# sitzikbs/Nesti-Net

Hardware: AMD Instinct MI355X
Metric: normals/sec (whole node), synthetic 100k-pt clouds (higher is better)
Workload: dtype f16x8c

## Files before the change

### nesti-net_amd/csrc/conv4n.hip

```cpp
#include <type_traits>

#include "kernels.h"
#include "mma.h"

namespace nesti {
namespace {

constexpr int kThreads4 = 512;
constexpr int kPts4 = 16;
constexpr int kTile4 = 1024;
constexpr int kBTap4 = 4 * kTile4;
constexpr int kABuf4 = 64 * kTile4;
constexpr int kEpiStride4 = 144;
constexpr int kEpi4 = 1024 * kEpiStride4;
template <int K> constexpr bool dba4() { return 2 * K * kBTap4 + 2 * kABuf4 <= 163840; }
template <int K> constexpr int lds4() {
  constexpr int loop = 2 * K * kBTap4 + (dba4<K>() ? 2 : 1) * kABuf4;
  return loop > kEpi4 ? loop : kEpi4;
}
constexpr unsigned kOob4 = 0x40000u;

typedef unsigned u32x4q_t __attribute__((ext_vector_type(4)));
typedef const __attribute__((address_space(3))) u32x4q_t* lds_u32x4q_ptr;
__device__ __forceinline__ uint4 lds128q(unsigned addr) {
  const u32x4q_t v = *(lds_u32x4q_ptr)(size_t)addr;
  return make_uint4(v.x, v.y, v.z, v.w);
}

typedef __attribute__((ext_vector_type(4))) float f32x4;
template <int DT> __device__ __forceinline__ void mma16(f32x4& acc, const uint4& a, const uint4& b);
template <> __device__ __forceinline__ void mma16<NESTI_BF16>(f32x4& acc, const uint4& a, const uint4& b) {
  acc = __builtin_amdgcn_mfma_f32_16x16x32_bf16(__builtin_bit_cast(bf16x8, a), __builtin_bit_cast(bf16x8, b), acc, 0, 0, 0);
}
template <> __device__ __forceinline__ void mma16<NESTI_F16>(f32x4& acc, const uint4& a, const uint4& b) {
  acc = __builtin_amdgcn_mfma_f32_16x16x32_f16(__builtin_bit_cast(f16x8, a), __builtin_bit_cast(f16x8, b), acc, 0, 0, 0);
}
template <> __device__ __forceinline__ void mma16<NESTI_F32>(f32x4& acc, const uint4& a, const uint4& b) {
  acc = __builtin_amdgcn_mfma_f32_16x16x4f32(__uint_as_float(a.x), __uint_as_float(b.x), acc, 0, 0, 0);
  acc = __builtin_amdgcn_mfma_f32_16x16x4f32(__uint_as_float(a.y), __uint_as_float(b.y), acc, 0, 0, 0);
  acc = __builtin_amdgcn_mfma_f32_16x16x4f32(__uint_as_float(a.z), __uint_as_float(b.z), acc, 0, 0, 0);
  acc = __builtin_amdgcn_mfma_f32_16x16x4f32(__uint_as_float(a.w), __uint_as_float(b.w), acc, 0, 0, 0);
}

__device__ __forceinline__ int swz4(int r) { return (0x78 >> (2 * ((r >> 2) & 3))) & 3; }

template <int DT, int K, bool X3>
__device__ __forceinline__ void conv4n_tile(const ConvParams& p, const unsigned bid, const int tid_in) {
  extern __shared__ __attribute__((aligned(16))) unsigned char smem[];
  constexpr int kEsz = (DT == NESTI_F32) ? 4 : 2;
  constexpr int NB = X3 ? 2 : 1;
  constexpr int LO = (K - 1) / 2;
  constexpr int NR = K * K;
  constexpr bool PREF = !X3 && K == 4;
  static_assert(K >= 2 && K <= 5, "kernel edge");
  constexpr bool DBA = dba4<K>();
  constexpr int kSlotB = K * kBTap4;
  constexpr int kAOff = 2 * kSlotB;
  constexpr int APR = NR >= 6 ? 4 : 2;
  constexpr int APP = 8 / APR;
  static_assert(lds4<K>() <= 163840, "LDS budget");

  const int tid = tid_in, lane = tid & 63;
  const int wave = __builtin_amdgcn_readfirstlane(tid >> 6);
  const int cw = wave & 3, h = wave >> 2;

  const int xcd = bid & 7, grp = bid >> 3;
  const int n_tile = grp % p.n_tiles;
  const int m_tile = (grp / p.n_tiles) * 8 + xcd;
  if (m_tile >= p.m_tiles) return;
  int npts = p.npoints;
  if (p.npoints_ptr) npts = min(npts, *p.npoints_ptr);
  const int p0 = m_tile * kPts4;
  if (p0 >= npts) return;
  const int np_here = min(kPts4, npts - p0);

  const unsigned lds0 = (unsigned)(size_t)(lptr_t)smem;
  const unsigned char* in_b = reinterpret_cast<const unsigned char*>(p.in) + ((size_t)p0 * 64 * p.in_cstride + p.in_coff) * kEsz;
  const unsigned char* w_tile = reinterpret_cast<const unsigned char*>(p.wpk) + (size_t)n_tile * p.n_chunks * (K * K * K) * kBTap4;

  const int st_row = lane >> 2;
  const int st_slot = (lane & 3) ^ swz4(st_row);
  const bool st_ok = st_row < np_here;
  const size_t st_off = (size_t)st_row * 64 * p.in_cstride * kEsz +
                        (X3 ? (size_t)((st_slot & 1) * 16 + (st_slot >> 1) * (2 * kSplitGroup)) : (size_t)st_slot * 16);
  auto stage_a = [&](int c, int buf, int q0, int nq) __attribute__((always_inline)) {
    const size_t coff = X3 ? (size_t)(c >> 2) * (2 * kPairPlanes * kSplitGroup) + (size_t)(c & 3) * 32
                           : p.in_pair ? (size_t)(c >> 1) * (2 * kPairPlanes * kSplitGroup) + (size_t)(c & 1) * 64 : (size_t)c * 64;
#pragma unroll
    for (int qq = 0; qq < nq; ++qq) {
      const int s = wave * 8 + q0 + qq;
      const int x = s & 3, z = (s >> 2) & 3, y = ((s >> 4) - z) & 3;
      const int v = 16 * z + 4 * y + x;
      if (st_ok) glds16(in_b + (size_t)v * p.in_cstride * kEsz + coff + st_off, lds0 + kAOff + buf * kABuf4 + s * kTile4);
    }
  };
  auto stage_b = [&](int g) __attribute__((always_inline)) {
    const unsigned char* src = w_tile + (size_t)g * kSlotB;
    for (int pid = wave; pid < 4 * K; pid += 8) glds16(src + pid * 1024 + lane * 16, lds0 + (g & 1) * kSlotB + pid * 1024);
  };

  const int r16 = lane & 15, kb = lane >> 4;
  const unsigned frag = (unsigned)(r16 * 64 + ((kb ^ swz4(r16)) << 4));
  const unsigned a_lane = lds0 + kAOff + frag;
  unsigned b_lane[NB];
  if (X3) {
    b_lane[0] = lds0 + (unsigned)(r16 * 64 + (((kb & 1) ^ swz4(r16)) << 4));
    b_lane[NB - 1] = kb < 2 ? lds0 + (unsigned)(r16 * 64 + (((2 + (kb & 1)) ^ swz4(r16)) << 4)) : kOob4;
  } else {
    b_lane[0] = lds0 + frag;
  }

  unsigned ymk = 0u, zmk = 0u;
#pragma unroll
  for (int d = 0; d < 5; ++d)
#pragma unroll
    for (int j = 0; j < 2; ++j) {
      const int z = 2 * h + j, y = (cw - z) & 3;
      if ((unsigned)(y + d - 2) < 4u) ymk |= 1u << (2 * d + j);
      if ((unsigned)(z + d - 2) < 4u) zmk |= 1u << (2 * d + j);
    }
  auto row_info = [&](int iz, int iy, int buf, unsigned& live, unsigned& abase) __attribute__((always_inline)) {
    const int dz = iz - LO, dy = iy - LO;
    live = (zmk >> (2 * (dz + 2))) & (ymk >> (2 * (dy + 2))) & 3u;
    const int tile0 = 4 * (4 * ((cw + dy + dz) & 3) + 2 * h + dz);
    abase = a_lane + (unsigned)(buf * kABuf4 + tile0 * kTile4);
  };

  f32x4 acc[2][4][4];
#pragma unroll
  for (int j = 0; j < 2; ++j)
#pragma unroll
    for (int x = 0; x < 4; ++x)
#pragma unroll
      for (int n = 0; n < 4; ++n)
#pragma unroll
        for (int r = 0; r < 4; ++r) acc[j][x][n][r] = 0.f;

  uint4 a[2][4], an[2][4], b[2][4][NB];
  auto load_a = [&](uint4 (&dst)[2][4], unsigned base) __attribute__((always_inline)) {
#pragma unroll
    for (int j = 0; j < 2; ++j)
#pragma unroll
      for (int x = 0; x < 4; ++x) dst[j][x] = lds128q(base + (4 * j + x) * kTile4);
  };
  auto load_b = [&](uint4 (&dst)[4][NB], unsigned off) __attribute__((always_inline)) {
#pragma unroll
    for (int n = 0; n < 4; ++n)
#pragma unroll
      for (int s = 0; s < NB; ++s) dst[n][s] = lds128q(b_lane[s] + off + n * kTile4);
  };

  const int G = p.n_chunks * NR;
  stage_a(0, 0, 0, 8);
  stage_b(0);
  stage_b(1);
  wait_vm0();
  __syncthreads();
  unsigned live_c, abase_c;
  row_info(0, 0, 0, live_c, abase_c);
  load_b(b[K & 1], 0u);
  if (PREF) load_a(an, abase_c);
  int c = 0, row = 0, iz = 0, iy = 0;
  for (int g = 0; g < G; ++g) {
    int cn = c, rown = row + 1, izn = iz, iyn = iy + 1;
    if (iyn == K) { iyn = 0; ++izn; }
    if (rown == NR) { rown = 0; izn = 0; iyn = 0; ++cn; }
    unsigned live_n = 0u, abase_n = abase_c;
    if (g + 1 < G) row_info(izn, iyn, DBA ? (cn & 1) : 0, live_n, abase_n);
    const bool stage_now = DBA && row < APR && c + 1 < p.n_chunks;
    if (stage_now) stage_a(c + 1, (c + 1) & 1, row * APP, APP);
    if (!PREF) {
      load_a(a, abase_c);
    } else {
#pragma unroll
      for (int j = 0; j < 2; ++j)
#pragma unroll
        for (int x = 0; x < 4; ++x) a[j][x] = an[j][x];
      load_a(an, abase_n);
    }
    const unsigned lv = live_c;
    const unsigned slot_off = (unsigned)((g & 1) * kSlotB), nslot_off = (unsigned)(((g + 1) & 1) * kSlotB);
#pragma unroll
    for (int u = 0; u < K; ++u) {
      const bool last = (u == K - 1);
      if ((K & 1) && u == 0) {
#pragma unroll
        for (int n = 0; n < 4; ++n)
#pragma unroll
          for (int s = 0; s < NB; ++s) b[0][n][s] = b[1][n][s];
      }
      uint4(&bc)[4][NB] = b[u & 1];
      uint4(&bn)[4][NB] = b[(u + 1) & 1];
      if (last) {
        __builtin_amdgcn_s_waitcnt(0xC07F);
        if (stage_now) asm volatile("s_waitcnt vmcnt(%0)" ::"n"(APP) : "memory");
        else wait_vm0();
        __builtin_amdgcn_s_barrier();
        if (g + 2 < G) stage_b(g + 2);
        if (!DBA && rown == 0 && g + 1 < G) {
          stage_a(cn, 0, 0, 8);
        }
      }
      load_b(bn, last ? nslot_off : slot_off + (unsigned)((u + 1) * kBTap4));
#pragma unroll
      for (int j = 0; j < 2; ++j) {
        if (__builtin_expect((lv & (1u << j)) != 0, 1)) {
#pragma unroll
          for (int x = 0; x < 4; ++x) {
            const int xs = x + u - LO;
            if (xs >= 0 && xs < 4) {
#pragma unroll
              for (int s = 0; s < NB; ++s)
#pragma unroll
                for (int n = 0; n < 4; ++n) mma16<DT>(acc[j][x][n], a[j][xs], bc[n][s]);
            }
          }
        }
      }
    }
    if (!DBA && rown == 0 && g + 1 < G) {
      wait_vm0();
      __builtin_amdgcn_s_barrier();
    }
    live_c = live_n;
    abase_c = abase_n;
    c = cn; row = rown; iz = izn; iy = iyn;
  }
  __builtin_amdgcn_s_waitcnt(0xC07F);
  __syncthreads();

  const int out_esz = p.out_f32 ? 4 : kEsz;
  const float act_floor = p.relu ? 0.f : -INFINITY;
  unsigned char* out_b = reinterpret_cast<unsigned char*>(p.out);
  unsigned char* mp_b = reinterpret_cast<unsigned char*>(p.mp_out);
  auto cvt_store8 = [&](unsigned char* base, long long row_elems, int col, const float4& f0, const float4& f1) __attribute__((always_inline)) {
    if (out_esz == 4) {
      float4* dst = reinterpret_cast<float4*>(base + (row_elems + col) * 4);
      dst[0] = f0;
      dst[1] = f1;
    } else {
      using E = Elem<DT == NESTI_F32 ? NESTI_BF16 : DT>;
      store_act8<E>(base, row_elems, col, f0, f1, p.split);
    }
  };
  auto epi_pass = [&](auto PP) __attribute__((always_inline)) {
    constexpr int pass = decltype(PP)::value;
    const int out_col0 = p.out_coff + n_tile * 64 + pass * 32;
#pragma unroll
    for (int n2 = 0; n2 < 2; ++n2) {
      const int n = 2 * pass + n2;
      const float bv = p.bias[n_tile * 64 + n * 16 + r16];
#pragma unroll
      for (int j = 0; j < 2; ++j) {
        const int z = 2 * h + j, y = (cw - z) & 3;
#pragma unroll
        for (int x = 0; x < 4; ++x) {
          const int v = 16 * z + 4 * y + x;
#pragma unroll
          for (int r = 0; r < 4; ++r) {
            const int row = (4 * kb + r) * 64 + v;
            *reinterpret_cast<float*>(smem + row * kEpiStride4 + (n2 * 16 + r16) * 4) = fmaxf(fmaf(acc[j][x][n][r], p.acc_scale, bv), act_floor);
          }
        }
      }
    }
    __syncthreads();
    if (p.mp_mode != 1) {
#pragma unroll 2
      for (int it = 0; it < 8; ++it) {
        const int item = it * kThreads4 + tid;
        const int row = item >> 2, seg = item & 3;
        const int ptl = row >> 6, vox = row & 63;
        if (ptl < np_here) {
          const float4 f0 = *reinterpret_cast<const float4*>(smem + row * kEpiStride4 + seg * 32);
          const float4 f1 = *reinterpret_cast<const float4*>(smem + row * kEpiStride4 + seg * 32 + 16);
          cvt_store8(out_b, ((long long)(p0 + ptl) * 64 + vox) * p.out_cstride, out_col0 + seg * 8, f0, f1);
        }
      }
    }
    if (p.mp_mode != 0) {
      const int cell = tid >> 2, seg = tid & 3;
      const int ptl = cell >> 3, cz = (cell >> 2) & 1, cy = (cell >> 1) & 1, cx = cell & 1;
      float4 m0 = make_float4(-INFINITY, -INFINITY, -INFINITY, -INFINITY), m1 = m0;
#pragma unroll
      for (int q = 0; q < 8; ++q) {
        const int row = ptl * 64 + (2 * cz + (q >> 2)) * 16 + (2 * cy + ((q >> 1) & 1)) * 4 + 2 * cx + (q & 1);
        const float4 f0 = *reinterpret_cast<const float4*>(smem + row * kEpiStride4 + seg * 32);
        const float4 f1 = *reinterpret_cast<const float4*>(smem + row * kEpiStride4 + seg * 32 + 16);
        m0.x = fmaxf(m0.x, f0.x); m0.y = fmaxf(m0.y, f0.y); m0.z = fmaxf(m0.z, f0.z); m0.w = fmaxf(m0.w, f0.w);
        m1.x = fmaxf(m1.x, f1.x); m1.y = fmaxf(m1.y, f1.y); m1.z = fmaxf(m1.z, f1.z); m1.w = fmaxf(m1.w, f1.w);
      }
      if (ptl < np_here)
        cvt_store8(mp_b, ((long long)(p0 + ptl) * 8 + (cz * 4 + cy * 2 + cx)) * p.mp_cstride, out_col0 + seg * 8, m0, m1);
    }
    __syncthreads();
  };
  epi_pass(std::integral_constant<int, 0>{});
  epi_pass(std::integral_constant<int, 1>{});
}

template <int DT, int K, bool X3, bool WALK>
__global__ __launch_bounds__(kThreads4) void conv4n_kernel(const ConvParams p) {
  if constexpr (!WALK) {
    conv4n_tile<DT, K, X3>(p, blockIdx.x, threadIdx.x);
  } else {
    unsigned n_blocks;
    {
      int npts = p.npoints;
      if (p.npoints_ptr) npts = min(npts, *p.npoints_ptr);
      const unsigned m_live = (unsigned)((npts + kPts4 - 1) / kPts4);
        n_blocks = (m_live + 7) / 8 * 8 * (unsigned)p.n_tiles;
    }
    for (unsigned bid = blockIdx.x; bid < n_blocks; bid += gridDim.x) {
      if (bid != blockIdx.x) __syncthreads();
      int tid = threadIdx.x;
      asm volatile("" : "+v"(tid));
      conv4n_tile<DT, K, X3>(p, bid, tid);
    }
  }
}

template <int DT, int K, bool X3, bool WALK>
int launch_conv4n_one_w(const ConvParams& p, hipStream_t stream) {
  constexpr int kMaxDevices = 64;
  static bool attr_set[kMaxDevices] = {};
  int dev = 0;
  NESTI_CHECK_HIP(hipGetDevice(&dev));
  if (dev < 0 || dev >= kMaxDevices || !attr_set[dev]) {
    NESTI_CHECK_HIP(hipFuncSetAttribute(reinterpret_cast<const void*>(&conv4n_kernel<DT, K, X3, WALK>),
                                        hipFuncAttributeMaxDynamicSharedMemorySize, lds4<K>()));
    if (dev >= 0 && dev < kMaxDevices) attr_set[dev] = true;
  }
  const int groups = (p.m_tiles + 7) / 8;
  const unsigned n_blocks = (unsigned)(groups * 8 * p.n_tiles);
  dim3 grid(WALK ? std::min(n_blocks, p.walk > 1 ? (unsigned)p.walk : kWalkGrid) : n_blocks), block(kThreads4);
  hipLaunchKernelGGL((conv4n_kernel<DT, K, X3, WALK>), grid, block, lds4<K>(), stream, p);
  NESTI_CHECK_HIP(hipGetLastError());
  return 0;
}

template <int DT, int K, bool X3>
int launch_conv4n_one(const ConvParams& p, hipStream_t stream) {
  return p.walk ? launch_conv4n_one_w<DT, K, X3, true>(p, stream) : launch_conv4n_one_w<DT, K, X3, false>(p, stream);
}

template <int DT>
int launch_conv4n_dt(const ConvParams& p, int k, hipStream_t stream) {
  if constexpr (DT != NESTI_F32) {
    if (p.x3native) {
      if (k == 2) return launch_conv4n_one<DT, 2, true>(p, stream);
      if (k == 4) return launch_conv4n_one<DT, 4, true>(p, stream);
      NESTI_FAIL("launch_conv4n: the pair K loop is built for k = 2 and k = 4");
    }
  }
  if (p.x3native) NESTI_FAIL("launch_conv4n: the pair K loop is for the 16-bit kernels");
  if (k == 2) return launch_conv4n_one<DT, 2, false>(p, stream);
  if (k == 3) return launch_conv4n_one<DT, 3, false>(p, stream);
  if (k == 4) return launch_conv4n_one<DT, 4, false>(p, stream);
  if (k == 5) return launch_conv4n_one<DT, 5, false>(p, stream);
  NESTI_FAIL("launch_conv4n: kernel size must be 2 .. 5");
}

}

int launch_conv4n(const ConvParams& p, int dtype, int k, hipStream_t stream) {
  if (p.m_tiles <= 0 || p.n_tiles <= 0) return 0;
  if (p.log2S != 2 || p.s_real) NESTI_FAIL("launch_conv4n: the 4^3 volume only");
  if (k < 2 || k > 5 || p.n_taps != k * k * k || p.tap_k != k) NESTI_FAIL("launch_conv4n: all k^3 taps (k = 2 .. 5) must be present");
  for (int t = 0; t < p.n_taps; ++t) {
    const int lo = (k - 1) / 2;
    if (p.tap[t][0] != t / (k * k) - lo || p.tap[t][1] != (t / k) % k - lo || p.tap[t][2] != t % k - lo)
      NESTI_FAIL("launch_conv4n: taps must be in (dz, dy, dx) order, x fastest");
  }
  if (p.point_index) NESTI_FAIL("launch_conv4n: no input gather (k^3 layers never read the routed MuPS tensor)");
  if (p.pool_k > 1 || p.split_tile != p.n_tiles) NESTI_FAIL("launch_conv4n: no fused avg-pool / merged layers");
  if (p.mp_mode == 2) NESTI_FAIL("launch_conv4n: max-pool mode 2 is conv1's (a 1x1x1 layer)");
  if (p.mp_mode != 0 && !p.mp_out) NESTI_FAIL("launch_conv4n: fused max-pool needs an output");
  if (dtype == NESTI_BF16) return launch_conv4n_dt<NESTI_BF16>(p, k, stream);
  if (dtype == NESTI_F16) return launch_conv4n_dt<NESTI_F16>(p, k, stream);
  if (dtype == NESTI_F32) return launch_conv4n_dt<NESTI_F32>(p, k, stream);
  NESTI_FAIL("launch_conv4n: unsupported dtype");
}

}
```

### nesti-net_amd/csrc/conv8n.hip

```cpp
#include <string.h>

#include <mutex>

#include <type_traits>

#include "kernels.h"
#include "mma.h"

namespace nesti {
namespace {

constexpr int kThreadsN = 512;
constexpr int kPtsN = 4;
constexpr int kTileN = 2048;
constexpr int kBTileN = 2 * kTileN;
constexpr int kAOffN = 65536;
constexpr unsigned kOobN = 0x40000u;
constexpr int kEpiStrideN = 144;

typedef unsigned u32x4n_t __attribute__((ext_vector_type(4)));
typedef const __attribute__((address_space(3))) u32x4n_t* lds_u32x4n_ptr;
__device__ __forceinline__ uint4 lds128n(unsigned addr) {
  const u32x4n_t v = *(lds_u32x4n_ptr)(size_t)addr;
  return make_uint4(v.x, v.y, v.z, v.w);
}

typedef unsigned u32x2n_t __attribute__((ext_vector_type(2)));
typedef const __attribute__((address_space(3))) u32x2n_t* lds_u32x2n_ptr;
typedef const __attribute__((address_space(3))) unsigned* lds_u32n_ptr;
template <bool X6>
__device__ __forceinline__ uint4 lds_hi16n(unsigned addr) {
  if constexpr (X6) {
    const u32x2n_t d = *(lds_u32x2n_ptr)(size_t)addr;
    const unsigned sc = *(lds_u32n_ptr)(size_t)(addr + 8u);
    return make_uint4(d.x, d.y, sc, 0u);
  } else {
    return lds128n(addr);
  }
}

template <int K> constexpr int lds_bytes_n() { return kAOffN + 8 * (4 + (K - 1) / 2) * kTileN; }

typedef int i32x8n_t __attribute__((ext_vector_type(8)));

template <int DT, int K, int MODE>
__device__ __forceinline__ void conv8n_tile(const ConvParams& p, const unsigned bid, const int tid_in) {
  constexpr bool X3 = MODE == 1, X8 = MODE >= 2, X6 = MODE == 3;
  static_assert(!X8 || DT == NESTI_F16, "the FP8 cross-term loop is an f16 pair-mode variant");
  extern __shared__ __attribute__((aligned(16))) unsigned char smem[];
  constexpr int kEsz = (DT == NESTI_F32) ? 4 : 2;
  constexpr int LO = (K - 1) / 2;
  constexpr int NG = K * K;
  constexpr int NZ = 4 + LO;
  constexpr int R = (K == 3) ? 2 : 1;
  constexpr int NS = (K == 3) ? 2 : 3;
  constexpr int AHEAD = NS - 1;
  constexpr int kSlot = R * K * kBTileN;
  constexpr int NSR = (NG + R - 1) / R;
  static_assert(NS * kSlot <= kAOffN, "weight slots must fit below the input chunk");
  static_assert((K & 1) == 1, "the weight-fragment ping-pong assumes an odd number of taps per row");

  const int tid = tid_in, lane = tid & 63;
  const int wave = __builtin_amdgcn_readfirstlane(tid >> 6);

  const int xcd = bid & 7, grp = bid >> 3;
  const int per_m = 2 * p.n_tiles;
  const int sub = grp % per_m;
  const int n_pair = sub >> 1, half = sub & 1;
  const int m_tile = (grp / per_m) * 8 + xcd;
  if (m_tile >= p.m_tiles) return;
  int npts = p.npoints;
  if (p.npoints_ptr) npts = min(npts, *p.npoints_ptr);
  const int p0 = m_tile * kPtsN;
  if (p0 >= npts) return;
  const int np_here = min(kPtsN, npts - p0);
  const int z0 = 4 * half;
  const int zlo = half ? 8 - NZ : 0;

  const unsigned lds0 = (unsigned)(size_t)(lptr_t)smem;
  const unsigned char* in_b = reinterpret_cast<const unsigned char*>(p.in) +
                              ((size_t)p0 * 512 * p.in_cstride + p.in_coff) * kEsz;
  const unsigned char* w_tile = reinterpret_cast<const unsigned char*>(p.wpk) +
                                (size_t)n_pair * p.n_chunks * (K * K * K) * kBTileN;

  const int st_row = lane >> 2;
  unsigned a_voff[2];
  bool a_ok[2];
  bool a_is8[2];
  const unsigned char* aux_b = nullptr;
  if constexpr (X8) aux_b = reinterpret_cast<const unsigned char*>(p.aux8_in) + (size_t)p0 * 512 * p.aux8_stride;
#pragma unroll
  for (int h = 0; h < 2; ++h) {
    const int pt = 2 * h + (st_row >> 3), x = st_row & 7;
    const int kslot = (lane & 3) ^ pt;
    a_voff[h] = (unsigned)((pt * 512 + x) * p.in_cstride * kEsz + (X3 ? (kslot & 1) * 16 + (kslot >> 1) * (2 * kSplitGroup) : kslot * 16));
    a_is8[h] = X8 && kslot >= 2;
    if (a_is8[h]) a_voff[h] = (unsigned)((pt * 512 + x) * p.aux8_stride + (kslot - 2) * kSplitGroup);
    a_ok[h] = pt < np_here;
  }
  auto stage_a = [&](int c) __attribute__((always_inline)) {
#pragma unroll
    for (int jz = 0; jz < NZ; ++jz) {
      const int zp = zlo + jz, yp = (wave - zp) & 7;
      if constexpr (X8) {
        const size_t off16 = (size_t)((zp * 64 + yp * 8) * p.in_cstride) * kEsz + (size_t)(c >> 2) * (2 * kPairPlanes * kSplitGroup) + (size_t)(c & 3) * 32;
        const size_t off8 = (size_t)(zp * 64 + yp * 8) * p.aux8_stride + (size_t)(c >> 2) * (2 * kSplitGroup) + (size_t)(c & 3) * 16;
#pragma unroll
        for (int h = 0; h < 2; ++h)
          if (a_ok[h]) glds16((a_is8[h] ? aux_b + off8 : in_b + off16) + a_voff[h], lds0 + kAOffN + (wave * NZ + jz) * kTileN + h * 1024);
      } else {
      const unsigned char* src = in_b + (size_t)((zp * 64 + yp * 8) * p.in_cstride) * kEsz +
                                 (X3 ? (size_t)(c >> 2) * (2 * kPairPlanes * kSplitGroup) + (size_t)(c & 3) * 32
                                     : p.in_pair ? (size_t)(c >> 1) * (2 * kPairPlanes * kSplitGroup) + (size_t)(c & 1) * 64 : (size_t)c * 64);
#pragma unroll
      for (int h = 0; h < 2; ++h)
        if (a_ok[h]) glds16(src + a_voff[h], lds0 + kAOffN + (wave * NZ + jz) * kTileN + h * 1024);
      }
    }
  };
  auto stage_b = [&](int c, int sr, int slot) __attribute__((always_inline)) {
    const unsigned char* src = w_tile + ((size_t)c * (K * K * K) + (size_t)sr * R * K) * kBTileN;
    const int pieces = 4 * K * min(R, NG - sr * R);
    for (int pid = wave; pid < pieces; pid += 8)
      glds16(src + pid * 1024 + lane * 16, lds0 + slot * kSlot + pid * 1024);
  };

  const int l31 = lane & 31, khalf = lane >> 5;
  const int pt = l31 >> 3, rx = l31 & 7;
  const int a_sw = (khalf ^ pt) & 3, b_sw = (khalf ^ (l31 >> 2)) & 3;
  const unsigned a_lane = lds0 + kAOffN + (unsigned)((pt * 8 + rx) * 64 + (a_sw << 4));
  const unsigned b_lane = lds0 + (unsigned)(l31 * 64 + (b_sw << 4));
  const unsigned a_d1 = (a_sw & 2) ? (unsigned)-32 : 32u, b_d1 = (b_sw & 2) ? (unsigned)-32 : 32u;

  unsigned ymask_pack = 0u, zmask_pack = 0u;
#pragma unroll
  for (int d = 0; d < K; ++d) {
    unsigned my = 0, mz = 0;
#pragma unroll
    for (int j = 0; j < 4; ++j) {
      const int y = (wave - z0 - j) & 7, z = z0 + j;
      if ((unsigned)(y + d - LO) < 8u) my |= 1u << j;
      if ((unsigned)(z + d - LO) < 8u) mz |= 1u << j;
    }
    ymask_pack |= my << (4 * d);
    zmask_pack |= mz << (4 * d);
  }
  unsigned pa[K];
#pragma unroll
  for (int d = 0; d < K; ++d) pa[d] = ((unsigned)(rx + d - LO) < 8u) ? a_lane + (unsigned)((d - LO) * 64) : kOobN;
  unsigned dslot_a = 0u, a8_d1 = 0u, b8k = 0u, b8_d1 = 0u;
  if constexpr (X8) {
    const int bkey = (l31 >> 2) & 3;
    dslot_a = (unsigned)((((2 ^ pt) & 3) - a_sw) * 16);
    a8_d1 = (unsigned)((((3 ^ pt) & 3) - ((2 ^ pt) & 3)) * 16);
    b8k = lds0 + (unsigned)(l31 * 64 + (((2 ^ bkey) & 3) << 4) + khalf * kBTileN);
    b8_d1 = (unsigned)((((3 ^ bkey) & 3) - ((2 ^ bkey) & 3)) * 16);
  }
  auto mask_of = [&](int dzi, int dyi) __attribute__((always_inline)) -> unsigned {
    return (zmask_pack >> (4 * dzi)) & (ymask_pack >> (4 * dyi)) & 0xfu;
  };
  auto base_of = [&](int dzi, int dyi) __attribute__((always_inline)) -> int {
    return (((wave + dyi + dzi - 2 * LO) & 7) * NZ + (z0 - zlo + dzi - LO)) * kTileN;
  };

  f32x16 acc[4][2];
#pragma unroll
  for (int j = 0; j < 4; ++j)
#pragma unroll
    for (int n = 0; n < 2; ++n)
#pragma unroll
      for (int r = 0; r < 16; ++r) acc[j][n][r] = 0.f;

  uint4 a[4][2], b[2][2][2];
  auto load_b = [&](uint4 (&dst)[2][2], unsigned src) __attribute__((always_inline)) {
#pragma unroll
    for (int n = 0; n < 2; ++n) {
      dst[n][0] = lds128n(src + n * kTileN);
      dst[n][1] = lds128n(src + n * kTileN + b_d1);
    }
  };
  auto tile_mma = [&](int j, const uint4 (&bc)[2][2]) __attribute__((always_inline)) {
    if (X3) {
      mma<DT>(acc[j][0], a[j][0], bc[0][0]);
      mma<DT>(acc[j][1], a[j][0], bc[1][0]);
      mma<DT>(acc[j][0], a[j][1], bc[0][0]);
      mma<DT>(acc[j][1], a[j][1], bc[1][0]);
      mma<DT>(acc[j][0], a[j][0], bc[0][1]);
      mma<DT>(acc[j][1], a[j][0], bc[1][1]);
    } else {
      mma<DT>(acc[j][0], a[j][0], bc[0][0]);
      mma<DT>(acc[j][1], a[j][0], bc[1][0]);
      mma<DT>(acc[j][0], a[j][1], bc[0][1]);
      mma<DT>(acc[j][1], a[j][1], bc[1][1]);
#ifdef CONV8N_DOUBLE_MMA
      mma<DT>(acc[j][0], a[j][0], bc[0][1]);
      mma<DT>(acc[j][1], a[j][0], bc[1][1]);
      mma<DT>(acc[j][0], a[j][1], bc[0][0]);
      mma<DT>(acc[j][1], a[j][1], bc[1][0]);
#endif
    }
  };
  auto row = [&](unsigned mask_g, unsigned mask_n, int base_g, int base_n, unsigned boff_g, unsigned boff_n,
                 bool pair_end) __attribute__((always_inline)) {
#pragma unroll
    for (int u = 0; u < K; ++u) {
      const bool last_u = (u == K - 1);
      unsigned m_mm = mask_g, m_rd = last_u ? mask_n : mask_g;
      asm volatile("" : "+s"(m_mm), "+s"(m_rd));
      const unsigned nb0 = pa[last_u ? 0 : u + 1] + (unsigned)(last_u ? base_n : base_g);
      const unsigned nb1 = nb0 + a_d1;
      const unsigned bsrc = b_lane + (last_u ? boff_n : boff_g + (unsigned)((u + 1) * kBTileN));
      if (R > 1 && last_u && pair_end) {
        __builtin_amdgcn_s_waitcnt(0xC07F);
        wait_vm0();
        __builtin_amdgcn_s_barrier();
      }
      if (u == 0) {
#pragma unroll
        for (int n = 0; n < 2; ++n) { b[0][n][0] = b[1][n][0]; b[0][n][1] = b[1][n][1]; }
      }
      uint4(&bc)[2][2] = b[u & 1];
      uint4(&bn)[2][2] = b[(u + 1) & 1];
      load_b(bn, bsrc);
#pragma unroll
      for (int j = 0; j < 4; ++j) {
        if (__builtin_expect((m_mm & (1u << j)) != 0, 1)) tile_mma(j, bc);
        a[j][0] = lds128n(nb0 + j * kTileN);
        a[j][1] = lds128n(nb1 + j * kTileN);
      }
    }
    if (R == 1) {
      wait_vm0();
      __builtin_amdgcn_s_barrier();
    }
  };


  uint4 a8[2][2], b8[2][2];
  int sc_a = p.x8_scale_a, sc_b = p.x8_scale_b;
  if constexpr (!X6) asm volatile("" : "+v"(sc_a), "+v"(sc_b));
  auto mma8 = [&](f32x16& c, const uint4 (&av)[2], const uint4 (&bv)[2]) __attribute__((always_inline)) {
    const i32x8n_t a_ = {(int)av[0].x, (int)av[0].y, (int)av[0].z, (int)av[0].w, (int)av[1].x, (int)av[1].y, (int)av[1].z, (int)av[1].w};
    const i32x8n_t b_ = {(int)bv[0].x, (int)bv[0].y, (int)bv[0].z, (int)bv[0].w, (int)bv[1].x, (int)bv[1].y, (int)bv[1].z, (int)bv[1].w};
    if constexpr (X6) {
      c = __builtin_amdgcn_mfma_scale_f32_32x32x64_f8f6f4(a_, b_, c, 2, 2, 0, (int)av[1].z, 0, (int)bv[1].z);
    } else {
      c = __builtin_amdgcn_mfma_scale_f32_32x32x64_f8f6f4(a_, b_, c, 0, 0, 0, sc_a, 0, sc_b);
    }
  };
  auto a8_same = [&](int d0, unsigned base) __attribute__((always_inline)) -> unsigned {
    return (khalf ? pa[d0 + 1] : pa[d0]) + dslot_a + base;
  };
  auto row8 = [&](const int T, unsigned mask_g, unsigned mask_n, int base_g, int base_n, unsigned boff_g, unsigned boff_n, bool more,
                  bool pair_end) __attribute__((always_inline)) {
    unsigned selA = 0u, selB = 0u, lv = 0u;
    if (T == 0) {
      selA = (khalf ? pa[0] + (unsigned)base_n : pa[K - 1] + (unsigned)base_g) + dslot_a;
      selB = khalf ? (more ? b8k - (unsigned)kBTileN + boff_n : kOobN) : b8k + (unsigned)((K - 1) * kBTileN) + boff_g;
      lv = khalf ? mask_n : mask_g;
    }
    auto a8_x = [&](int j) __attribute__((always_inline)) -> unsigned { return ((lv >> j) & 1u) ? selA : kOobN; };
    const unsigned m_mm = (unsigned)__builtin_amdgcn_readfirstlane((int)mask_g);
    const unsigned m_x = (unsigned)__builtin_amdgcn_readfirstlane((int)(mask_g | mask_n));
#pragma unroll
    for (int u = 0; u < K; ++u) {
      const bool last_u = (u == K - 1);
      const bool cross = T == 0 ? ((u & 1) || last_u) : (u >= 2 && !(u & 1));
      const bool xrow = T == 0 && last_u;
      const bool next_x = T == 0 && u == K - 2;
      const unsigned nb0 = pa[last_u ? 0 : u + 1] + (unsigned)(last_u ? base_n : base_g);
      const unsigned bsrc = b_lane + (last_u ? boff_n : boff_g + (unsigned)((u + 1) * kBTileN));
      if (R > 1 && last_u && pair_end) {
        __builtin_amdgcn_s_waitcnt(0xC07F);
        wait_vm0();
        __builtin_amdgcn_s_barrier();
      }
      const int d0 = u - 1;
      unsigned cb8 = 0u, nb8 = 0u, bsrc8 = 0u;
      if (cross) {
        if (!xrow) cb8 = a8_same(d0, (unsigned)base_g);
        if (!next_x) {
          const int nd0 = last_u ? (T == 0 ? 1 : 0) : u + 1;
          nb8 = a8_same(nd0, (unsigned)(last_u ? base_n : base_g));
          bsrc8 = b8k + (unsigned)(nd0 * kBTileN) + (last_u ? boff_n : boff_g);
        } else {
          bsrc8 = selB;
        }
      }
      unsigned m0 = m_mm, m1 = m_mm, m2 = xrow ? m_x : m_mm;
      asm volatile("" : "+s"(m0), "+s"(m1), "+s"(m2));
#pragma unroll
      for (int j = 0; j < 4; ++j)
        if (__builtin_expect((m0 & (1u << j)) != 0, 1)) mma<DT>(acc[j][0], a[j][0], b[0][0][0]);
      b[0][0][0] = lds128n(bsrc);
#pragma unroll
      for (int j = 0; j < 4; ++j) {
        if (__builtin_expect((m1 & (1u << j)) != 0, 1)) mma<DT>(acc[j][1], a[j][0], b[0][1][0]);
        a[j][0] = lds128n(nb0 + j * kTileN);
      }
      b[0][1][0] = lds128n(bsrc + kTileN);
      if (cross) {
#pragma unroll
        for (int j = 0; j < 4; ++j) {
          if (__builtin_expect((m2 & (1u << j)) != 0, 1)) {
            mma8(acc[j][0], a8[j & 1], b8[0]);
            mma8(acc[j][1], a8[j & 1], b8[1]);
          }
          const unsigned src8 = j < 2 ? (xrow ? a8_x(j + 2) : cb8) + (j + 2) * kTileN : (next_x ? a8_x(j - 2) : nb8) + (j - 2) * kTileN;
          a8[j & 1][0] = lds128n(src8);
          a8[j & 1][1] = lds_hi16n<X6>(src8 + a8_d1);
        }
      }
      if (cross) {
#pragma unroll
        for (int n = 0; n < 2; ++n) {
          b8[n][0] = lds128n(bsrc8 + n * kTileN);
          b8[n][1] = lds_hi16n<X6>(bsrc8 + b8_d1 + n * kTileN);
        }
      }
    }
    if (R == 1) {
      wait_vm0();
      __builtin_amdgcn_s_barrier();
    }
  };

  for (int c = 0; c < p.n_chunks; ++c) {
    __syncthreads();
    stage_a(c);
#pragma unroll
    for (int sr = 0; sr < AHEAD; ++sr) stage_b(c, sr, sr);
    wait_vm0();
    __syncthreads();
    {
      const unsigned m0 = mask_of(0, 0);
      const unsigned nb0 = pa[0] + (unsigned)base_of(0, 0);
      const unsigned nb1 = nb0 + a_d1;
      if constexpr (X8) {
        const unsigned nb8 = a8_same(0, (unsigned)base_of(0, 0));
#pragma unroll
        for (int n = 0; n < 2; ++n) {
          b[0][n][0] = lds128n(b_lane + n * kTileN);
          b8[n][0] = lds128n(b8k + n * kTileN);
          b8[n][1] = lds_hi16n<X6>(b8k + b8_d1 + n * kTileN);
        }
#pragma unroll
        for (int j = 0; j < 4; ++j) a[j][0] = lds128n(nb0 + j * kTileN);
#pragma unroll
        for (int j = 0; j < 2; ++j) {
          a8[j][0] = lds128n(nb8 + j * kTileN);
          a8[j][1] = lds_hi16n<X6>(nb8 + a8_d1 + j * kTileN);
        }
      } else {
      load_b(b[1], b_lane);
#pragma unroll
      for (int j = 0; j < 4; ++j)
        if (m0 & (1u << j)) {
          a[j][0] = lds128n(nb0 + j * kTileN);
          a[j][1] = lds128n(nb1 + j * kTileN);
        }
      }
    }
    int dzi = 0, dyi = 0, fill = AHEAD, fslot = AHEAD % NS, g = 0;
    unsigned boff = 0u;
    auto do_row = [&](const int T) __attribute__((always_inline)) {
      if (g % R == 0 && fill < NSR) {
        stage_b(c, fill, fslot);
        ++fill;
        fslot = (fslot + 1 == NS) ? 0 : fslot + 1;
      }
      const bool more = g + 1 < NG;
      int dzn = dzi, dyn = dyi + 1;
      if (dyn == K) { dyn = 0; ++dzn; }
      unsigned boff_n = (R > 1 && (g & 1) == 0) ? boff + (unsigned)(K * kBTileN) : (boff - (boff % kSlot)) + kSlot;
      if (boff_n >= (unsigned)(NS * kSlot)) boff_n = 0u;
      const unsigned mask_g = mask_of(dzi, dyi), mask_n = more ? mask_of(dzn, dyn) : 0u;
      const int base_g = base_of(dzi, dyi), base_n = more ? base_of(dzn, dyn) : 0;
      const bool pair_end = (g % R == R - 1) || !more;
      if constexpr (X8) row8(T, mask_g, mask_n, base_g, base_n, boff, boff_n, more, pair_end);
      else row(mask_g, mask_n, base_g, base_n, boff, boff_n, pair_end);
      dzi = dzn; dyi = dyn; boff = boff_n; ++g;
    };
    if constexpr (X8) {
      for (int gp = 0; gp < NG / 2; ++gp) {
        do_row(0);
        do_row(1);
      }
      do_row(0);
    } else {
      for (int gg = 0; gg < NG; ++gg) do_row(0);
    }
  }
  __builtin_amdgcn_s_waitcnt(0xC07F);
  __syncthreads();

  const int out_esz = p.out_f32 ? 4 : kEsz;
  const float act_floor = p.relu ? 0.f : -INFINITY;
  unsigned char* out_b = reinterpret_cast<unsigned char*>(p.out);
  unsigned char* mp_b = reinterpret_cast<unsigned char*>(p.mp_out);
  auto cvt_store8 = [&](unsigned char* base, long long row_elems, int col, const float4& f0, const float4& f1) __attribute__((always_inline)) {
    if (out_esz == 4) {
      float4* dst = reinterpret_cast<float4*>(base + (row_elems + col) * 4);
      dst[0] = f0;
      dst[1] = f1;
    } else {
      using E = Elem<DT == NESTI_F32 ? NESTI_BF16 : DT>;
      store_act8<E>(base, row_elems, col, f0, f1, p.split);
    }
  };
  auto epi_pass = [&](auto NN) __attribute__((always_inline)) {
    constexpr int n = decltype(NN)::value;
    const int n_tile = 2 * n_pair + n;
    const float bv = p.bias[n_tile * 32 + l31];
    const int out_col0 = p.out_coff + n_tile * 32;
#pragma unroll
    for (int j = 0; j < 4; ++j) {
      const int y = (wave - z0 - j) & 7;
#pragma unroll
      for (int r = 0; r < 16; ++r) {
        const int m = (r & 3) + 8 * (r >> 2) + 4 * khalf;
        const int row = ((((m >> 3) * 4 + j) * 8 + y) << 3) + (m & 7);
        *reinterpret_cast<float*>(smem + row * kEpiStrideN + l31 * 4) = fmaxf(fmaf(acc[j][n][r], p.acc_scale, bv), act_floor);
      }
    }
    __syncthreads();
    if (p.mp_mode != 1) {
#pragma unroll 2
      for (int it = 0; it < 8; ++it) {
        const int item = it * kThreadsN + tid;
        const int row = item >> 2, seg = item & 3;
        const int ptl = row >> 8, vox = z0 * 64 + (row & 255);
        if (ptl < np_here) {
          const float4 f0 = *reinterpret_cast<const float4*>(smem + row * kEpiStrideN + seg * 32);
          const float4 f1 = *reinterpret_cast<const float4*>(smem + row * kEpiStrideN + seg * 32 + 16);
          cvt_store8(out_b, ((long long)(p0 + ptl) * 512 + vox) * p.out_cstride, out_col0 + seg * 8, f0, f1);
        }
      }
    }
    if (p.mp_mode != 0) {
      const int cell = tid >> 2, seg = tid & 3;
      const int ptl = cell >> 5, cz = (cell >> 4) & 1, cy = (cell >> 2) & 3, cx = cell & 3;
      float4 m0 = make_float4(-INFINITY, -INFINITY, -INFINITY, -INFINITY), m1 = m0;
#pragma unroll
      for (int q = 0; q < 8; ++q) {
        const int row = ((ptl * 4 + 2 * cz + (q >> 2)) * 8 + 2 * cy + ((q >> 1) & 1)) * 8 + 2 * cx + (q & 1);
        const float4 f0 = *reinterpret_cast<const float4*>(smem + row * kEpiStrideN + seg * 32);
        const float4 f1 = *reinterpret_cast<const float4*>(smem + row * kEpiStrideN + seg * 32 + 16);
        m0.x = fmaxf(m0.x, f0.x); m0.y = fmaxf(m0.y, f0.y); m0.z = fmaxf(m0.z, f0.z); m0.w = fmaxf(m0.w, f0.w);
        m1.x = fmaxf(m1.x, f1.x); m1.y = fmaxf(m1.y, f1.y); m1.z = fmaxf(m1.z, f1.z); m1.w = fmaxf(m1.w, f1.w);
      }
      if (ptl < np_here) {
        const int ovox = ((2 * half + cz) * 4 + cy) * 4 + cx;
        cvt_store8(mp_b, ((long long)(p0 + ptl) * 64 + ovox) * p.mp_cstride, out_col0 + seg * 8, m0, m1);
      }
    }
    __syncthreads();
  };
  epi_pass(std::integral_constant<int, 0>{});
  epi_pass(std::integral_constant<int, 1>{});
}

template <int DT, int K, int MODE, bool WALK>
__global__ __launch_bounds__(kThreadsN) void conv8n_kernel(const ConvParams p) {
  if constexpr (!WALK) {
    conv8n_tile<DT, K, MODE>(p, blockIdx.x, threadIdx.x);
  } else {
    unsigned n_blocks;
    {
      int npts = p.npoints;
      if (p.npoints_ptr) npts = min(npts, *p.npoints_ptr);
      const unsigned m_live = (unsigned)((npts + kPtsN - 1) / kPtsN);
        n_blocks = (m_live + 7) / 8 * 8 * 2u * (unsigned)p.n_tiles;
    }
    for (unsigned bid = blockIdx.x; bid < n_blocks; bid += gridDim.x) {
      if (bid != blockIdx.x) __syncthreads();
      int tid = threadIdx.x;
      asm volatile("" : "+v"(tid));
      conv8n_tile<DT, K, MODE>(p, bid, tid);
    }
  }
}

template <int DT, int K, int MODE, bool WALK>
int launch_conv8n_one_w(const ConvParams& p, hipStream_t stream) {
  constexpr int kMaxDevices = 64;
  static bool attr_set[kMaxDevices] = {};
  int dev = 0;
  NESTI_CHECK_HIP(hipGetDevice(&dev));
  constexpr int lds = lds_bytes_n<K>();
  static_assert(lds <= 163840 && 1024 * kEpiStrideN <= lds, "LDS budget");
  if (dev < 0 || dev >= kMaxDevices || !attr_set[dev]) {
    NESTI_CHECK_HIP(hipFuncSetAttribute(reinterpret_cast<const void*>(&conv8n_kernel<DT, K, MODE, WALK>),
                                        hipFuncAttributeMaxDynamicSharedMemorySize, lds));
    if (dev >= 0 && dev < kMaxDevices) attr_set[dev] = true;
  }
  const int groups = (p.m_tiles + 7) / 8;
  const unsigned n_blocks = (unsigned)(groups * 8 * 2 * p.n_tiles);
  dim3 grid(WALK ? std::min(n_blocks, p.walk > 1 ? (unsigned)p.walk : kWalkGrid) : n_blocks), block(kThreadsN);
  hipLaunchKernelGGL((conv8n_kernel<DT, K, MODE, WALK>), grid, block, lds, stream, p);
  NESTI_CHECK_HIP(hipGetLastError());
  return 0;
}

template <int DT, int K, int MODE>
int launch_conv8n_one(const ConvParams& p, hipStream_t stream) {
  return p.walk ? launch_conv8n_one_w<DT, K, MODE, true>(p, stream) : launch_conv8n_one_w<DT, K, MODE, false>(p, stream);
}

template <int DT>
int launch_conv8n_dt(const ConvParams& p, int k, hipStream_t stream) {
  if constexpr (DT == NESTI_F16) {
    if (p.x8) {
      if (!p.aux8_in || p.aux8_stride <= 0 || !p.split) NESTI_FAIL("launch_conv8n: the FP8 cross-term loop needs the side buffer of e4m3 planes and pair outputs");
      if (p.x8_fmt == 6) {
        if (k == 5) return launch_conv8n_one<DT, 5, 3>(p, stream);
        if (k == 3) return launch_conv8n_one<DT, 3, 3>(p, stream);
      }
      if (k == 5) return launch_conv8n_one<DT, 5, 2>(p, stream);
      if (k == 3) return launch_conv8n_one<DT, 3, 2>(p, stream);
    }
  }
  if (p.x8) NESTI_FAIL("launch_conv8n: the FP8 cross-term loop is an f16 pair-mode variant");
  if constexpr (DT != NESTI_F32) {
    if (p.x3native && k == 5) return launch_conv8n_one<DT, 5, 1>(p, stream);
    if (p.x3native && k == 3) return launch_conv8n_one<DT, 3, 1>(p, stream);
  }
  if (p.x3native) NESTI_FAIL("launch_conv8n: the pair K loop is for the 16-bit kernels");
  if (k == 5) return launch_conv8n_one<DT, 5, 0>(p, stream);
  if (k == 3) return launch_conv8n_one<DT, 3, 0>(p, stream);
  NESTI_FAIL("launch_conv8n: kernel size must be 3 or 5");
}

__global__ void lds_oob_probe_kernel(unsigned* out, unsigned lds) {
  extern __shared__ __attribute__((aligned(16))) unsigned char smem[];
  for (unsigned i = threadIdx.x; i < lds / 4; i += blockDim.x) reinterpret_cast<unsigned*>(smem)[i] = 0xA5A50000u + i;
  __syncthreads();
  const uint4 v = lds128n(kOobN + 16u * threadIdx.x);
  const uint4 w = lds128n((unsigned)(size_t)(lptr_t)smem + 16u * threadIdx.x);
  atomicOr(&out[0], v.x | v.y | v.z | v.w);
  atomicOr(&out[1], w.x == 0xA5A50000u + 4u * threadIdx.x ? 0u : 1u);
}

}

int conv8_selftest() {
  constexpr int kMaxDevices = 64;
  static int state[kMaxDevices] = {};
  static std::mutex mu;
  std::lock_guard<std::mutex> lk(mu);
  int dev = 0;
  NESTI_CHECK_HIP(hipGetDevice(&dev));
  if (dev < 0 || dev >= kMaxDevices) NESTI_FAIL("conv8_selftest: device index out of range");
  if (state[dev] == 1) return 0;
  if (state[dev] == 0) {
    hipDeviceProp_t prop;
    NESTI_CHECK_HIP(hipGetDeviceProperties(&prop, dev));
    if (strncmp(prop.gcnArchName, "gfx950", 6) != 0) {
      state[dev] = 2;
    } else {
      unsigned* d = nullptr;
      unsigned h[2] = {1u, 1u};
      NESTI_CHECK_HIP(hipMalloc((void**)&d, 8));
      NESTI_CHECK_HIP(hipMemset(d, 0, 8));
      for (unsigned lds : {65536u, 147456u, 163840u}) {
        NESTI_CHECK_HIP(hipFuncSetAttribute(reinterpret_cast<const void*>(&lds_oob_probe_kernel),
                                            hipFuncAttributeMaxDynamicSharedMemorySize, (int)lds));
        hipLaunchKernelGGL(lds_oob_probe_kernel, dim3(1), dim3(256), lds, 0, d, lds);
      }
      NESTI_CHECK_HIP(hipMemcpy(h, d, 8, hipMemcpyDeviceToHost));
      (void)hipFree(d);
      state[dev] = (h[0] == 0u && h[1] == 0u) ? 1 : 2;
    }
  }
  if (state[dev] == 2)
    NESTI_FAIL("this device is not a gfx950 whose out-of-range LDS reads return zero: the 8^3 tap kernels (conv8n.hip) "
               "take their x padding from such reads and would compute wrong convolutions here");
  return 0;
}

int launch_conv8n(const ConvParams& p, int dtype, int k, hipStream_t stream) {
  if (p.m_tiles <= 0 || p.n_tiles <= 0) return 0;
  if (p.log2S != 3 || p.s_real) NESTI_FAIL("launch_conv8n: the 8^3 volume only");
  if (p.n_taps != k * k * k) NESTI_FAIL("launch_conv8n: all k^3 taps must be present");
  if (p.point_index) NESTI_FAIL("launch_conv8n: no input gather (k^3 layers never read the routed MuPS tensor)");
  if (p.pool_k > 1 || p.split_tile != p.n_tiles) NESTI_FAIL("launch_conv8n: no fused avg-pool / merged layers");
  if (p.mp_mode == 2) NESTI_FAIL("launch_conv8n: max-pool mode 2 is conv1's (a 1x1x1 layer)");
  if (p.mp_mode != 0 && !p.mp_out) NESTI_FAIL("launch_conv8n: fused max-pool needs an output");
  if (dtype == NESTI_BF16) return launch_conv8n_dt<NESTI_BF16>(p, k, stream);
  if (dtype == NESTI_F16) return launch_conv8n_dt<NESTI_F16>(p, k, stream);
  if (dtype == NESTI_F32) return launch_conv8n_dt<NESTI_F32>(p, k, stream);
  NESTI_FAIL("launch_conv8n: unsupported dtype");
}

}
```

### nesti-net_amd/csrc/mma.h

```cpp
#pragma once
#include "kernels.h"

namespace nesti {
namespace {

typedef __attribute__((ext_vector_type(8))) __bf16 bf16x8;
typedef __attribute__((ext_vector_type(8))) _Float16 f16x8;
typedef __attribute__((ext_vector_type(16))) float f32x16;

template <int DT> __device__ __forceinline__ void mma(f32x16& acc, const uint4& a, const uint4& b);
template <> __device__ __forceinline__ void mma<NESTI_BF16>(f32x16& acc, const uint4& a, const uint4& b) {
  acc = __builtin_amdgcn_mfma_f32_32x32x16_bf16(__builtin_bit_cast(bf16x8, a), __builtin_bit_cast(bf16x8, b), acc, 0, 0, 0);
}
template <> __device__ __forceinline__ void mma<NESTI_F16>(f32x16& acc, const uint4& a, const uint4& b) {
  acc = __builtin_amdgcn_mfma_f32_32x32x16_f16(__builtin_bit_cast(f16x8, a), __builtin_bit_cast(f16x8, b), acc, 0, 0, 0);
}
template <> __device__ __forceinline__ void mma<NESTI_F32>(f32x16& acc, const uint4& a, const uint4& b) {
  acc = __builtin_amdgcn_mfma_f32_32x32x2f32(__uint_as_float(a.x), __uint_as_float(b.x), acc, 0, 0, 0);
  acc = __builtin_amdgcn_mfma_f32_32x32x2f32(__uint_as_float(a.y), __uint_as_float(b.y), acc, 0, 0, 0);
  acc = __builtin_amdgcn_mfma_f32_32x32x2f32(__uint_as_float(a.z), __uint_as_float(b.z), acc, 0, 0, 0);
  acc = __builtin_amdgcn_mfma_f32_32x32x2f32(__uint_as_float(a.w), __uint_as_float(b.w), acc, 0, 0, 0);
}

typedef __attribute__((address_space(3))) unsigned char* lptr_t;

__device__ __forceinline__ void glds16(const unsigned char* src, unsigned lds_dst) {
  unsigned keep;
  asm volatile(
      "s_mov_b32 %0, m0\n\ts_mov_b32 m0, %2\n\ts_nop 0\n\tglobal_load_lds_dwordx4 %1, off\n\ts_mov_b32 m0, %0"
      : "=&s"(keep)
      : "v"(src), "s"(lds_dst)
      : "memory");
}
__device__ __forceinline__ void wait_vm0() { asm volatile("s_waitcnt vmcnt(0)" ::: "memory"); }

}
}
```

Before: 48780.

## Use 16x16x32 MFMA tiles in the f16 non-pair conv8n path

For f16 in mode 0, the conv8n tile now computes with 16x16x32 MFMA instructions and four f32x4 accumulators per output pair instead of 32x32x16. Lane-to-row mapping, swizzle keys and LDS fragment offsets are redefined for 16-lane rows, and the epilogue is rewritten to scatter the new accumulator layout. The mma16 helpers move into the shared header. The aim is to use an MFMA shape whose throughput or issue latency suits this loop better, at the cost of more instructions, a different LDS access pattern and an extra accumulator array that could raise register pressure.

```diff
diff --git a/nesti-net_amd/csrc/conv4n.hip b/nesti-net_amd/csrc/conv4n.hip
--- a/nesti-net_amd/csrc/conv4n.hip
+++ b/nesti-net_amd/csrc/conv4n.hip
@@ -25,21 +25,6 @@
 __device__ __forceinline__ uint4 lds128q(unsigned addr) {
   const u32x4q_t v = *(lds_u32x4q_ptr)(size_t)addr;
   return make_uint4(v.x, v.y, v.z, v.w);
-}
-
-typedef __attribute__((ext_vector_type(4))) float f32x4;
-template <int DT> __device__ __forceinline__ void mma16(f32x4& acc, const uint4& a, const uint4& b);
-template <> __device__ __forceinline__ void mma16<NESTI_BF16>(f32x4& acc, const uint4& a, const uint4& b) {
-  acc = __builtin_amdgcn_mfma_f32_16x16x32_bf16(__builtin_bit_cast(bf16x8, a), __builtin_bit_cast(bf16x8, b), acc, 0, 0, 0);
-}
-template <> __device__ __forceinline__ void mma16<NESTI_F16>(f32x4& acc, const uint4& a, const uint4& b) {
-  acc = __builtin_amdgcn_mfma_f32_16x16x32_f16(__builtin_bit_cast(f16x8, a), __builtin_bit_cast(f16x8, b), acc, 0, 0, 0);
-}
-template <> __device__ __forceinline__ void mma16<NESTI_F32>(f32x4& acc, const uint4& a, const uint4& b) {
-  acc = __builtin_amdgcn_mfma_f32_16x16x4f32(__uint_as_float(a.x), __uint_as_float(b.x), acc, 0, 0, 0);
-  acc = __builtin_amdgcn_mfma_f32_16x16x4f32(__uint_as_float(a.y), __uint_as_float(b.y), acc, 0, 0, 0);
-  acc = __builtin_amdgcn_mfma_f32_16x16x4f32(__uint_as_float(a.z), __uint_as_float(b.z), acc, 0, 0, 0);
-  acc = __builtin_amdgcn_mfma_f32_16x16x4f32(__uint_as_float(a.w), __uint_as_float(b.w), acc, 0, 0, 0);
 }
 
 __device__ __forceinline__ int swz4(int r) { return (0x78 >> (2 * ((r >> 2) & 3))) & 3; }
diff --git a/nesti-net_amd/csrc/conv8n.hip b/nesti-net_amd/csrc/conv8n.hip
--- a/nesti-net_amd/csrc/conv8n.hip
+++ b/nesti-net_amd/csrc/conv8n.hip
@@ -46,6 +46,7 @@
 template <int DT, int K, int MODE>
 __device__ __forceinline__ void conv8n_tile(const ConvParams& p, const unsigned bid, const int tid_in) {
   constexpr bool X3 = MODE == 1, X8 = MODE >= 2, X6 = MODE == 3;
+  constexpr bool M16 = MODE == 0 && DT == NESTI_F16;
   static_assert(!X8 || DT == NESTI_F16, "the FP8 cross-term loop is an f16 pair-mode variant");
   extern __shared__ __attribute__((aligned(16))) unsigned char smem[];
   constexpr int kEsz = (DT == NESTI_F32) ? 4 : 2;
@@ -126,11 +127,14 @@
   };
 
   const int l31 = lane & 31, khalf = lane >> 5;
-  const int pt = l31 >> 3, rx = l31 & 7;
-  const int a_sw = (khalf ^ pt) & 3, b_sw = (khalf ^ (l31 >> 2)) & 3;
+  const int lr = M16 ? (lane & 15) : l31;
+  const int ks = M16 ? (0x9C >> (2 * (lane >> 4))) & 3 : khalf;
+  const int pt = lr >> 3, rx = lr & 7;
+  const int a_sw = (ks ^ pt) & 3, b_sw = (ks ^ (lr >> 2)) & 3;
   const unsigned a_lane = lds0 + kAOffN + (unsigned)((pt * 8 + rx) * 64 + (a_sw << 4));
-  const unsigned b_lane = lds0 + (unsigned)(l31 * 64 + (b_sw << 4));
-  const unsigned a_d1 = (a_sw & 2) ? (unsigned)-32 : 32u, b_d1 = (b_sw & 2) ? (unsigned)-32 : 32u;
+  const unsigned b_lane = lds0 + (unsigned)(lr * 64 + (b_sw << 4));
+  const unsigned a_d1 = (M16 ? 1024u : 0u) + ((a_sw & 2) ? (unsigned)-32 : 32u);
+  const unsigned b_d1 = M16 ? 1024u : (b_sw & 2) ? (unsigned)-32 : 32u;
 
   unsigned ymask_pack = 0u, zmask_pack = 0u;
 #pragma unroll
@@ -164,12 +168,16 @@
   };
 
   f32x16 acc[4][2];
+  f32x4 acc4[4][2][4];
 #pragma unroll
   for (int j = 0; j < 4; ++j)
 #pragma unroll
-    for (int n = 0; n < 2; ++n)
+    for (int n = 0; n < 2; ++n) {
 #pragma unroll
       for (int r = 0; r < 16; ++r) acc[j][n][r] = 0.f;
+#pragma unroll
+      for (int q = 0; q < 4; ++q) acc4[j][n][q] = f32x4{0.f, 0.f, 0.f, 0.f};
+    }
 
   uint4 a[4][2], b[2][2][2];
   auto load_b = [&](uint4 (&dst)[2][2], unsigned src) __attribute__((always_inline)) {
@@ -180,13 +188,18 @@
     }
   };
   auto tile_mma = [&](int j, const uint4 (&bc)[2][2]) __attribute__((always_inline)) {
-    if (X3) {
+    if constexpr (X3) {
       mma<DT>(acc[j][0], a[j][0], bc[0][0]);
       mma<DT>(acc[j][1], a[j][0], bc[1][0]);
       mma<DT>(acc[j][0], a[j][1], bc[0][0]);
       mma<DT>(acc[j][1], a[j][1], bc[1][0]);
       mma<DT>(acc[j][0], a[j][0], bc[0][1]);
       mma<DT>(acc[j][1], a[j][0], bc[1][1]);
+    } else if constexpr (M16) {
+#pragma unroll
+      for (int h = 0; h < 2; ++h)
+#pragma unroll
+        for (int q = 0; q < 4; ++q) mma16<DT>(acc4[j][h][q], a[j][h], bc[q >> 1][q & 1]);
     } else {
       mma<DT>(acc[j][0], a[j][0], bc[0][0]);
       mma<DT>(acc[j][1], a[j][0], bc[1][0]);
@@ -411,16 +424,37 @@
   auto epi_pass = [&](auto NN) __attribute__((always_inline)) {
     constexpr int n = decltype(NN)::value;
     const int n_tile = 2 * n_pair + n;
-    const float bv = p.bias[n_tile * 32 + l31];
     const int out_col0 = p.out_coff + n_tile * 32;
-#pragma unroll
-    for (int j = 0; j < 4; ++j) {
-      const int y = (wave - z0 - j) & 7;
-#pragma unroll
-      for (int r = 0; r < 16; ++r) {
-        const int m = (r & 3) + 8 * (r >> 2) + 4 * khalf;
-        const int row = ((((m >> 3) * 4 + j) * 8 + y) << 3) + (m & 7);
-        *reinterpret_cast<float*>(smem + row * kEpiStrideN + l31 * 4) = fmaxf(fmaf(acc[j][n][r], p.acc_scale, bv), act_floor);
+    if constexpr (M16) {
+#pragma unroll
+      for (int k = 0; k < 2; ++k) {
+        const int col = 16 * k + (lane & 15);
+        const float bv = p.bias[n_tile * 32 + col];
+#pragma unroll
+        for (int j = 0; j < 4; ++j) {
+          const int y = (wave - z0 - j) & 7;
+#pragma unroll
+          for (int h = 0; h < 2; ++h)
+#pragma unroll
+            for (int r = 0; r < 4; ++r) {
+              const int m = 16 * h + 4 * (lane >> 4) + r;
+              const int row = ((((m >> 3) * 4 + j) * 8 + y) << 3) + (m & 7);
+              *reinterpret_cast<float*>(smem + row * kEpiStrideN + col * 4) =
+                  fmaxf(fmaf(acc4[j][h][2 * n + k][r], p.acc_scale, bv), act_floor);
+            }
+        }
+      }
+    } else {
+      const float bv = p.bias[n_tile * 32 + l31];
+#pragma unroll
+      for (int j = 0; j < 4; ++j) {
+        const int y = (wave - z0 - j) & 7;
+#pragma unroll
+        for (int r = 0; r < 16; ++r) {
+          const int m = (r & 3) + 8 * (r >> 2) + 4 * khalf;
+          const int row = ((((m >> 3) * 4 + j) * 8 + y) << 3) + (m & 7);
+          *reinterpret_cast<float*>(smem + row * kEpiStrideN + l31 * 4) = fmaxf(fmaf(acc[j][n][r], p.acc_scale, bv), act_floor);
+        }
       }
     }
     __syncthreads();
diff --git a/nesti-net_amd/csrc/mma.h b/nesti-net_amd/csrc/mma.h
--- a/nesti-net_amd/csrc/mma.h
+++ b/nesti-net_amd/csrc/mma.h
@@ -7,6 +7,7 @@
 typedef __attribute__((ext_vector_type(8))) __bf16 bf16x8;
 typedef __attribute__((ext_vector_type(8))) _Float16 f16x8;
 typedef __attribute__((ext_vector_type(16))) float f32x16;
+typedef __attribute__((ext_vector_type(4))) float f32x4;
 
 template <int DT> __device__ __forceinline__ void mma(f32x16& acc, const uint4& a, const uint4& b);
 template <> __device__ __forceinline__ void mma<NESTI_BF16>(f32x16& acc, const uint4& a, const uint4& b) {
@@ -20,6 +21,20 @@
   acc = __builtin_amdgcn_mfma_f32_32x32x2f32(__uint_as_float(a.y), __uint_as_float(b.y), acc, 0, 0, 0);
   acc = __builtin_amdgcn_mfma_f32_32x32x2f32(__uint_as_float(a.z), __uint_as_float(b.z), acc, 0, 0, 0);
   acc = __builtin_amdgcn_mfma_f32_32x32x2f32(__uint_as_float(a.w), __uint_as_float(b.w), acc, 0, 0, 0);
+}
+
+template <int DT> __device__ __forceinline__ void mma16(f32x4& acc, const uint4& a, const uint4& b);
+template <> __device__ __forceinline__ void mma16<NESTI_BF16>(f32x4& acc, const uint4& a, const uint4& b) {
+  acc = __builtin_amdgcn_mfma_f32_16x16x32_bf16(__builtin_bit_cast(bf16x8, a), __builtin_bit_cast(bf16x8, b), acc, 0, 0, 0);
+}
+template <> __device__ __forceinline__ void mma16<NESTI_F16>(f32x4& acc, const uint4& a, const uint4& b) {
+  acc = __builtin_amdgcn_mfma_f32_16x16x32_f16(__builtin_bit_cast(f16x8, a), __builtin_bit_cast(f16x8, b), acc, 0, 0, 0);
+}
+template <> __device__ __forceinline__ void mma16<NESTI_F32>(f32x4& acc, const uint4& a, const uint4& b) {
+  acc = __builtin_amdgcn_mfma_f32_16x16x4f32(__uint_as_float(a.x), __uint_as_float(b.x), acc, 0, 0, 0);
+  acc = __builtin_amdgcn_mfma_f32_16x16x4f32(__uint_as_float(a.y), __uint_as_float(b.y), acc, 0, 0, 0);
+  acc = __builtin_amdgcn_mfma_f32_16x16x4f32(__uint_as_float(a.z), __uint_as_float(b.z), acc, 0, 0, 0);
+  acc = __builtin_amdgcn_mfma_f32_16x16x4f32(__uint_as_float(a.w), __uint_as_float(b.w), acc, 0, 0, 0);
 }
 
 typedef __attribute__((address_space(3))) unsigned char* lptr_t;
```

After: 50640 (median of 6 runs). 1.04x the previous value.
